# chubbymaggie/syzkaller

Measured on AMD Instinct MI355X. Metric: signal elems triaged/sec (Diff+Merge), higher is better.
Workload: dtype u32

## Files before the change

syzkaller_amd/csrc/agg.hip:

```cpp
#include <algorithm>
#include <utility>
#include <vector>

#include "internal.h"

namespace syz {

constexpr uint32_t kAggThreads = 1024;
constexpr uint32_t kAggSlots = 7424;
constexpr uint32_t kAggBW = 4;
using KBucket = uint4;
constexpr uint32_t kAggBuckets = kAggSlots / kAggBW;
constexpr uint32_t kAggNoSlot = 0xFFFFFFFFu;
static_assert(kAggRegion == kAggSlots, "distinct-list region per partition (internal.h)");
constexpr uint32_t kAggLimit = kAggSlots * 4 / 5;
static_assert(kAggLimit == kAggLimitRecs, "internal.h mirror");
constexpr double kAggTargetLoad = 0.4;
constexpr double kAggTargetLoadEntry = 0.6;
constexpr uint64_t kMinItems = 2048;
constexpr uint32_t kAggEmpty = 0xFFFFFFFFu;
constexpr uint32_t kAggNone = 0xFFFFFFFFu;
constexpr uint32_t kAggOverflow = 0xFFFFFFFFu;
constexpr uint32_t kAggMinBits = 3, kAggMaxBits = 11;
constexpr uint32_t kAggMaxParts = 1u << kAggMaxBits;
constexpr uint32_t kAggTile = 18432;
constexpr uint32_t kAggGroup = 8;
constexpr uint32_t kAggU = 4, kAggD = 2;

struct AggGeom {
	uint32_t pbits;
	uint32_t ibits;
	__host__ __device__ uint32_t rbits() const { return 32 - pbits; }
	__host__ __device__ uint32_t cbits() const { return pbits - 2; }
	__host__ __device__ uint32_t items_per_chunk_log2() const { return cbits() - ibits; }
	__host__ __device__ uint32_t part(uint32_t h) const { return h >> (32 - pbits); }
	__host__ __device__ uint32_t meta(uint32_t level, uint64_t serial) const
	{
		return (level << cbits()) | ((uint32_t)serial & ((1u << cbits()) - 1));
	}
	__host__ __device__ uint32_t rec(uint32_t h, uint32_t meta) const { return (h << pbits) | meta; }
	__host__ __device__ uint32_t resid(uint32_t r) const { return r >> pbits; }
	__host__ __device__ uint32_t level(uint32_t r) const { return (r >> cbits()) & 3; }
	__host__ __device__ uint32_t local(uint32_t r) const { return r & ((1u << cbits()) - 1); }
};

__device__ __forceinline__ uint32_t agg_home_bucket(uint32_t key, const AggGeom& g)
{
	return __umulhi(key << g.pbits, kAggBuckets);
}

__device__ __forceinline__ uint32_t lds_flag(uint32_t* f)
{
	return __hip_atomic_load(f, __ATOMIC_RELAXED, __HIP_MEMORY_SCOPE_WORKGROUP);
}
__device__ __forceinline__ void lds_flag_set(uint32_t* f)
{
	__hip_atomic_store(f, 1u, __ATOMIC_RELAXED, __HIP_MEMORY_SCOPE_WORKGROUP);
}

__device__ __forceinline__ uint32_t bucket_find(uint4 B, uint32_t e)
{
	return B.x == e ? 0 : B.y == e ? 1 : B.z == e ? 2 : B.w == e ? 3 : 4;
}

__device__ __forceinline__ uint32_t bucket_first_empty(uint4 B)
{
	return B.x == kAggEmpty ? 0 : B.y == kAggEmpty ? 1 : B.z == kAggEmpty ? 2 : B.w == kAggEmpty ? 3 : 4;
}

__device__ uint32_t agg_find_insert(KBucket* kb, uint32_t e, uint32_t b, KBucket B, uint32_t* s_ovf, uint32_t& ins)
{
	uint32_t* keys = reinterpret_cast<uint32_t*>(kb);
	for (uint32_t step = 0; step < kAggBuckets;) {
		const uint32_t f = bucket_find(B, e);
		if (f < kAggBW)
			return b * kAggBW + f;
		const uint32_t j = bucket_first_empty(B);
		if (j == kAggBW) {
			b = b + 1 == kAggBuckets ? 0 : b + 1;
			B = kb[b];
			step++;
			continue;
		}
		const uint32_t i = b * kAggBW + j;
		const uint32_t key = atomicCAS(&keys[i], kAggEmpty, e);
		if (key == kAggEmpty) {
			ins++;
			return i;
		}
		if (key == e)
			return i;
		B = kb[b];
	}
	lds_flag_set(s_ovf);
	return kAggNoSlot;
}

struct CellGroup {
	uint64_t ch0;
	uint32_t bnd[kAggGroup + 1];
	__device__ void load(const uint32_t* __restrict__ ot, uint64_t nchunks, uint64_t gi)
	{
		ch0 = gi * kAggGroup;
#pragma unroll
		for (uint32_t i = 0; i <= kAggGroup; i++)
			bnd[i] = ot[min<uint64_t>(ch0 + i, nchunks)];
	}
	__device__ uint32_t serial(uint32_t j, uint32_t r, const AggGeom& g) const
	{
		uint32_t chunk = (uint32_t)ch0;
#pragma unroll
		for (uint32_t i = 1; i < kAggGroup; i++)
			chunk += j >= bnd[i];
		return (chunk << g.cbits()) | g.local(r);
	}
};

template <bool kShard>
__global__ __launch_bounds__(kAggThreads) void k_agg_count(const uint32_t* __restrict__ sigs,
                                                           const uint64_t* __restrict__ call_start,
                                                           const uint32_t* __restrict__ call_len, uint64_t c0,
                                                           uint64_t c1, AggGeom g, AggSrc x, uint32_t* counts)
{
	__shared__ uint32_t h[kAggMaxParts];
	auto add = [&](uint32_t e) {
		if (!kShard || owner_of(e, x.nshards) == x.shard)
			atomicAdd(&h[g.part(fmix32(e))], 1u);
	};
	const uint32_t P = 1u << g.pbits, cb = g.ibits;
	const uint32_t w = threadIdx.x >> 6, nw = blockDim.x >> 6, lane = lane_id();
	const uint64_t ncalls = c1 - c0, nchunks = (ncalls + (1ull << cb) - 1) >> cb;
	for (uint64_t ch = blockIdx.x; ch < nchunks; ch += gridDim.x) {
		for (uint32_t i = threadIdx.x; i < P; i += blockDim.x)
			h[i] = 0;
		__syncthreads();
		const uint64_t ce = min<uint64_t>(ncalls, (ch + 1) << cb);
		for (uint64_t s = (ch << cb) + w; s < ce; s += nw) {
			const uint64_t c = c0 + s, start = call_start[c];
			const uint32_t len = call_len[c];
			uint32_t j = lane;
			for (; j + 192 < len; j += 256) {
				const uint32_t a = sigs[start + j], b = sigs[start + j + 64], d = sigs[start + j + 128],
				               f = sigs[start + j + 192];
				add(a);
				add(b);
				add(d);
				add(f);
			}
			for (; j < len; j += 64)
				add(sigs[start + j]);
		}
		__syncthreads();
		for (uint32_t i = threadIdx.x; i < P; i += blockDim.x)
			counts[ch * P + i] = h[i];
		__syncthreads();
	}
}

__device__ __forceinline__ uint32_t block_excl_scan_1k(uint32_t v, uint32_t* out)
{
	__shared__ uint32_t wsum[16];
	const uint32_t lane = lane_id(), w = threadIdx.x >> 6, nw = blockDim.x >> 6;
	uint32_t x = v;
#pragma unroll
	for (int o = 1; o < 64; o <<= 1) {
		const uint32_t y = __shfl_up(x, o, 64);
		if (lane >= (uint32_t)o)
			x += y;
	}
	if (lane == 63)
		wsum[w] = x;
	__syncthreads();
	uint32_t pre = 0, tot = 0;
	for (uint32_t i = 0; i < nw; i++) {
		pre += i < w ? wsum[i] : 0;
		tot += wsum[i];
	}
	__syncthreads();
	*out = pre + x - v;
	return tot;
}

__global__ __launch_bounds__(1024) void k_agg_scan_chunks(const uint32_t* counts, uint64_t nitems, uint32_t ilog,
                                                          uint32_t P, uint32_t* offs, uint32_t* offsT, uint64_t* totals)
{
	const uint32_t p = blockIdx.x;
	const uint64_t nchunks = (nitems + (1ull << ilog) - 1) >> ilog;
	uint32_t* ot = offsT + (uint64_t)p * (nchunks + 1);
	uint64_t run = 0;
	for (uint64_t b0 = 0; b0 < nitems; b0 += blockDim.x) {
		const uint64_t b = b0 + threadIdx.x;
		const uint32_t v = b < nitems ? counts[b * P + p] : 0;
		uint32_t ex;
		const uint32_t tot = block_excl_scan_1k(v, &ex);
		if (b < nitems) {
			offs[b * P + p] = (uint32_t)(run + ex);
			if ((b & ((1ull << ilog) - 1)) == 0)
				ot[b >> ilog] = (uint32_t)(run + ex);
		}
		run += tot;
	}
	if (threadIdx.x == 0) {
		totals[p] = run;
		ot[nchunks] = (uint32_t)run;
	}
}

__global__ __launch_bounds__(1024) void k_agg_scan_totals(const uint64_t* totals, uint32_t P, uint64_t* rec_base)
{
	__shared__ uint64_t wsum[16];
	const uint32_t lane = lane_id(), w = threadIdx.x >> 6, i0 = threadIdx.x * 2;
	const uint64_t a = i0 < P ? totals[i0] : 0, b = i0 + 1 < P ? totals[i0 + 1] : 0;
	uint64_t x = a + b;
#pragma unroll
	for (int o = 1; o < 64; o <<= 1) {
		const uint64_t y = __shfl_up(x, o, 64);
		if (lane >= (uint32_t)o)
			x += y;
	}
	if (lane == 63)
		wsum[w] = x;
	__syncthreads();
	uint64_t pre = 0, tot = 0;
	for (uint32_t k = 0; k < 16; k++) {
		pre += k < w ? wsum[k] : 0;
		tot += wsum[k];
	}
	const uint64_t ex = pre + x - (a + b);
	if (i0 < P)
		rec_base[i0] = ex;
	if (i0 + 1 < P)
		rec_base[i0 + 1] = ex + a;
	if (threadIdx.x == 0)
		rec_base[P] = tot;
}

constexpr uint32_t kScatChunkMax = 1u << (kAggMaxBits - 2);
constexpr uint32_t kScatWaves = kAggThreads / 64;

constexpr uint32_t kScat3K = 16;
constexpr uint32_t kScat3KEntry = 10;
constexpr uint32_t kScat3Fill = 85;
constexpr uint32_t kScatPer = 12;
constexpr uint32_t kScatPerEntry = 10;
constexpr uint32_t kBlk = 16;
constexpr uint32_t kDummyLines = 2048;
typedef uint32_t scat_v4u __attribute__((ext_vector_type(4)));

struct CapCells {
	const uint64_t* base;
	const uint32_t* cap;
	uint32_t* cnt;
	uint32_t* ovf;
	uint64_t nchunks;
	uint32_t* dummy;
	const uint64_t* sizes = nullptr;
	const uint32_t* tiles = nullptr;
	bool split = false;
	uint32_t tile = 1024;
};

constexpr uint32_t kScat3Tile = kScat3K * 64, kScat3TileEntry = kScat3KEntry * 64;
__host__ __device__ inline uint64_t scat3_tiles(uint32_t len, uint32_t tile)
{
	return (len + tile - 1) / tile;
}
__device__ inline bool scat3_takes(uint64_t recs, uint32_t tiles, uint32_t tile)
{
	return recs * 100 >= (uint64_t)tiles * tile * kScat3Fill;
}

template <bool kOn>
struct PrioLevels {
	uint8_t lvl[kOn ? 256 : 1];
	__device__ __forceinline__ void load(const LevelMap& lm, uint32_t nthreads)
	{
		if (kOn) {
			for (uint32_t i = threadIdx.x; i < 256; i += nthreads)
				lvl[i] = lm.lvl[i];
		}
	}
	__device__ __forceinline__ uint32_t level(uint32_t pv, bool kept, bool& bad) const
	{
		const uint32_t lv = lvl[kOn ? pv : 0];
		bad |= kept && lv == 0xff;
		return lv & 3;
	}
	static __device__ __forceinline__ void report(bool bad, const AggSrc& x)
	{
		if (kOn && x.bad_level && __ballot(bad) && lane_id() == 0)
			atomicOr(x.bad_level, 1u);
	}
};

struct CallTable {
	uint64_t start[kScatChunkMax];
	uint32_t len[kScatChunkMax];
	uint16_t meta[kScatChunkMax];
	template <bool kEntry>
	__device__ __forceinline__ void load(const uint64_t* __restrict__ call_start, const uint32_t* __restrict__ call_len,
	                                     const uint8_t* __restrict__ call_prio, const LevelMap& lm, const AggGeom& g,
	                                     uint64_t c0, uint64_t cbeg, uint32_t nc)
	{
		for (uint32_t i = threadIdx.x; i < nc; i += blockDim.x) {
			const uint64_t c = c0 + cbeg + i;
			start[i] = call_start[c];
			len[i] = call_len[c];
			meta[i] = (uint16_t)g.meta(kEntry ? 0 : lm.lvl[call_prio[c]], cbeg + i);
		}
	}
	__device__ __forceinline__ uint32_t call_of(uint32_t w, uint32_t loc) const { return w + (loc >> 24) * kScatWaves; }
	template <bool kEntry, uint32_t kPer>
	__device__ __forceinline__ uint32_t fetch(uint32_t w, uint32_t lane, uint32_t nc, uint32_t& wc, uint32_t& wo,
	                                          const uint32_t* __restrict__ sigs, const AggSrc& x, uint32_t (&ev)[kPer],
	                                          uint32_t (&loc)[kPer], uint32_t (&pv)[kEntry ? kPer : 1]) const
	{
		constexpr uint32_t kQuota = kPer * 64;
		uint32_t q = 0;
		while (q < kQuota && wc < nc) {
			const uint32_t ln = len[wc], m = min(kQuota - q, ln - wo);
			const uint32_t tag = ((wc - w) / kScatWaves) << 24;
			if (q == 0) {
#pragma unroll
				for (uint32_t u = 0; u < kPer; u++)
					loc[u] = tag | wo;
			}
#pragma unroll
			for (uint32_t u = 0; u < kPer; u++) {
				const uint32_t i = u * 64 + lane;
				loc[u] = i >= q && i < q + m ? tag | (wo + i - q) : loc[u];
			}
			q += m;
			wo += m;
			if (wo == ln) {
				wc += kScatWaves;
				wo = 0;
			}
		}
		if (q) {
#pragma unroll
			for (uint32_t u = 0; u < kPer; u++) {
				const uint64_t a = start[call_of(w, loc[u])] + (loc[u] & 0xFFFFFFu);
				ev[u] = __builtin_nontemporal_load(&sigs[a]);
				if (kEntry)
					pv[kEntry ? u : 0] = (uint8_t)__builtin_nontemporal_load(&x.elem_prio[a]);
			}
		}
		return q;
	}
};

template <bool kEntry>
__global__ __launch_bounds__(kAggThreads) void k_agg_scatter(const uint32_t* __restrict__ sigs,
                                                             const uint64_t* __restrict__ call_start,
                                                             const uint32_t* __restrict__ call_len,
                                                             const uint8_t* __restrict__ call_prio, LevelMap lm,
                                                             uint64_t c0, uint64_t c1, AggGeom g, AggSrc x,
                                                             const uint32_t* __restrict__ offs,
                                                             const uint64_t* __restrict__ rec_base, uint32_t* recs)
{
	constexpr uint32_t kQuota = kAggTile / kScatWaves, kPer = kQuota / 64;
	static_assert(kQuota % 64 == 0, "tile quota per wave");
	__shared__ uint32_t t_rec[kAggTile];
	__shared__ uint16_t t_part[kAggTile];
	__shared__ uint64_t cur[kAggMaxParts];
	__shared__ uint32_t hist[kAggMaxParts], pos[kAggMaxParts];
	__shared__ CallTable calls;
	__shared__ PrioLevels<kEntry> levels;
	const uint32_t P = 1u << g.pbits, cb = g.cbits(), ib = g.ibits;
	levels.load(lm, blockDim.x);
	const uint32_t w = threadIdx.x >> 6, lane = lane_id();
	const uint64_t ncalls = c1 - c0, nitems = (ncalls + (1ull << ib) - 1) >> ib;
	const uint32_t per_t = (P + blockDim.x - 1) / blockDim.x;
	bool badlv = false;
	for (uint64_t ch = blockIdx.x; ch < nitems; ch += gridDim.x) {
		const uint64_t cbeg = ch << ib;
		const uint32_t nc = (uint32_t)min<uint64_t>(ncalls - cbeg, 1ull << ib);
		for (uint32_t i = threadIdx.x; i < P; i += blockDim.x) {
			cur[i] = rec_base[i] + offs[ch * P + i];
			hist[i] = 0;
		}
		calls.load<kEntry>(call_start, call_len, call_prio, lm, g, c0, cbeg, nc);
		__syncthreads();
		uint32_t wc = w, wo = 0;
		uint32_t ev[kPer], loc[kPer], pv[kEntry ? kPer : 1];
		auto fetch = [&]() { return calls.fetch<kEntry>(w, lane, nc, wc, wo, sigs, x, ev, loc, pv); };
		uint32_t n = fetch();
		for (;;) {
#pragma unroll
			for (uint32_t u = 0; u < kPer; u++) {
				const uint32_t i = u * 64 + lane;
				const bool keep = i < n && (!kEntry || x.nshards == 1 || owner_of(ev[u], x.nshards) == x.shard);
				if (keep) {
					const uint32_t h = fmix32(ev[u]), p = g.part(h);
					const uint32_t r = atomicAdd(&hist[p], 1u);
					uint32_t meta = calls.meta[calls.call_of(w, loc[u])];
					if (kEntry)
						meta |= levels.level(pv[kEntry ? u : 0], true, badlv) << cb;
					ev[u] = g.rec(h, meta);
					loc[u] = p | (r << 16);
				} else {
					loc[u] = ~0u;
				}
			}
			__syncthreads();
			uint32_t hsum = 0;
			for (uint32_t q = 0; q < per_t; q++) {
				const uint32_t i = threadIdx.x * per_t + q;
				hsum += i < P ? hist[i] : 0;
			}
			uint32_t ex;
			const uint32_t nt = block_excl_scan_1k(hsum, &ex);
			for (uint32_t q = 0; q < per_t; q++) {
				const uint32_t i = threadIdx.x * per_t + q;
				if (i < P) {
					pos[i] = ex;
					cur[i] -= ex;
					ex += hist[i];
				}
			}
			__syncthreads();
#pragma unroll
			for (uint32_t u = 0; u < kPer; u++) {
				if (loc[u] != ~0u) {
					const uint32_t p = loc[u] & 0xFFFFu, d = pos[p] + (loc[u] >> 16);
					t_rec[d] = ev[u];
					t_part[d] = (uint16_t)p;
				}
			}
			n = fetch();
			__syncthreads();
			for (uint32_t d = threadIdx.x; d < nt; d += blockDim.x)
				recs[cur[t_part[d]] + d] = t_rec[d];
			__syncthreads();
			for (uint32_t i = threadIdx.x; i < P; i += blockDim.x) {
				cur[i] += pos[i] + hist[i];
				hist[i] = 0;
			}
			if (!__syncthreads_or(n != 0))
				break;
		}
	}
	PrioLevels<kEntry>::report(badlv, x);
}

struct ScatLane {
	uint32_t w, lane;
	uint32_t seq = 0;
	bool spilled = false;
};
struct ScatItem {
	uint32_t* recs;
	uint64_t base;
	uint32_t cap;
};
template <uint32_t kB>
struct ScatBlocks {
	static_assert(kB == 16 || kB == 32, "block of 64 or 128 B");
	static constexpr uint32_t kMaxP = kB == 16 ? 2048 : 1024;
	static_assert(kMaxP * kB * 4 == 128 * 1024 && kMaxP <= kAggMaxParts, "128 KB of blocks");
	static constexpr uint32_t kG = 64 / kB;
	static constexpr uint32_t kLB = kB / 4, kGF = 64 / kLB;
	static constexpr uint32_t kShare = (kMaxP + kAggThreads - 1) / kAggThreads;
	alignas(16) uint32_t buf[kMaxP * kB];
	uint32_t fillc[kMaxP + 1];
	uint32_t written[kMaxP + 1];
	uint16_t flist[kShare * kAggThreads];
	uint32_t s_or[2][kScatWaves];

	__device__ __forceinline__ void reset(uint32_t P)
	{
		for (uint32_t i = threadIdx.x; i < P; i += kAggThreads) {
			fillc[i] = 0;
			written[i] = 0;
		}
	}
	__device__ __forceinline__ bool wg_or(ScatLane& t, bool pred)
	{
		uint32_t* r = s_or[t.seq++ & 1];
		const bool any = __ballot(pred) != 0;
		if (t.lane == 0)
			r[t.w] = any;
		__syncthreads();
		return __ballot(r[t.lane & (kScatWaves - 1)] != 0) != 0;
	}
	template <uint32_t M>
	__device__ __forceinline__ uint32_t place(const uint32_t (&rec)[M], const uint32_t (&pt)[M], uint32_t pend)
	{
		uint32_t sl[M];
#pragma unroll
		for (uint32_t u = 0; u < M; u++)
			sl[u] = (pend >> u) & 1 ? atomicAdd(&fillc[pt[u]], 1u) : kB;
#pragma unroll
		for (uint32_t u = 0; u < M; u++) {
			if (sl[u] < kB) {
				buf[pt[u] * kB + sl[u]] = rec[u];
				pend &= ~(1u << u);
			}
		}
		return pend;
	}
	__device__ __forceinline__ void flush(ScatLane& t, uint32_t P, const ScatItem& it, uint32_t* dummy)
	{
		const uint32_t fgrp = t.lane / kLB, fq = t.lane % kLB;
		uint16_t* wl = flist + t.w * kShare * 64;
		uint32_t nw = 0;
#pragma unroll
		for (uint32_t i = 0; i < kShare; i++) {
			const uint32_t p = i * kAggThreads + t.w * 64 + t.lane;
			const bool f = p < P && fillc[p] >= kB;
			const uint64_t m = __ballot(f);
			if (f)
				wl[nw + lane_rank(m)] = (uint16_t)p;
			nw += (uint32_t)__popcll(m);
		}
		for (uint32_t jb = 0; jb < nw; jb += kGF) {
			const bool ok = jb + fgrp < nw;
			const uint32_t pp = wl[min(jb + fgrp, nw - 1)];
			const uint32_t wr = written[pp];
			const scat_v4u v = *reinterpret_cast<const scat_v4u*>(&buf[pp * kB + fq * 4]);
			const bool fits = wr + kB <= it.cap;
			t.spilled |= ok && !fits;
			uint32_t* d = ok && fits ? it.recs + it.base + (uint64_t)pp * it.cap + wr
			                         : dummy + (blockIdx.x % (kDummyLines * kBlk / kB)) * kB;
			*reinterpret_cast<scat_v4u*>(d + fq * 4) = v;
			__builtin_amdgcn_wave_barrier();
			if (fq == 0 && ok) {
				written[pp] = wr + kB;
				fillc[pp] = 0;
			}
		}
	}
	template <uint32_t M>
	__device__ __forceinline__ void scatter_tile(ScatLane& t, uint32_t P, const ScatItem& it, uint32_t* dummy,
	                                             const uint32_t (&rec)[M], const uint32_t (&pt)[M], uint32_t pend)
	{
		for (;;) {
			pend = place(rec, pt, pend);
			const bool more = wg_or(t, pend != 0);
			flush(t, P, it, dummy);
			if (!more)
				break;
			__syncthreads();
		}
	}
	__device__ __forceinline__ void finish(ScatLane& t, uint32_t P, const ScatItem& it, const CapCells& cc, uint64_t ch)
	{
		const uint32_t grp = t.lane / kB, slot = t.lane & (kB - 1);
		for (uint32_t p = t.w * kG + grp; p < P; p += kScatWaves * kG) {
			const uint32_t c = fillc[p], wr = written[p];
			if (wr + c > it.cap)
				t.spilled = true;
			else if (slot < c)
				it.recs[it.base + (uint64_t)p * it.cap + wr + slot] = buf[p * kB + slot];
			if (slot == 0)
				cc.cnt[(uint64_t)p * cc.nchunks + ch] = min(wr + c, it.cap);
		}
		if (t.spilled)
			*cc.ovf = 1u;
		__syncthreads();
	}
};

template <bool kEntry, uint32_t kB>
__global__ __launch_bounds__(kAggThreads, 4) void k_agg_scatter_blk(const uint32_t* __restrict__ sigs,
                                                                    const uint64_t* __restrict__ call_start,
                                                                    const uint32_t* __restrict__ call_len,
                                                                    const uint8_t* __restrict__ call_prio, LevelMap lm,
                                                                    uint64_t c0, uint64_t c1, AggGeom g, AggSrc x,
                                                                    CapCells cc, uint32_t* recs)
{
	constexpr uint32_t kPer = kEntry ? kScatPerEntry : kScatPer;
// ... 63 lines not shown
		return;
	bool badlv = false;
	levels.load(lm, kAggThreads);
	for (uint64_t ch = blockIdx.x; ch < nchunks; ch += gridDim.x) {
		const uint64_t cbeg = ch << g.ibits;
		const uint32_t nc = (uint32_t)min<uint64_t>(ncalls - cbeg, 1ull << g.ibits);
		if (cc.split && !scat3_takes(cc.sizes[ch], cc.tiles[ch], cc.tile))
			continue;
		const ScatItem it{recs, cc.base[ch], cc.cap[ch]};
		blocks.reset(P);
		__syncthreads();
		uint32_t j = w, wo = 0, clen = 0, cmeta = 0;
		uint64_t cstart = 0;
		auto open_call = [&]() {
			while (j < nc) {
				const uint64_t c = c0 + cbeg + j;
				clen = call_len[c];
				if (clen) {
					cstart = call_start[c];
					const uintptr_t pa = (uintptr_t)(call_prio + c);
					const uint32_t word =
					    *(const __attribute__((address_space(4))) uint32_t*)(pa & ~(uintptr_t)3);
					cmeta = g.meta(kEntry ? 0 : levels.lvl[(word >> (8 * (pa & 3))) & 0xFF], cbeg + j);
					return;
				}
				j += kScatWaves;
			}
		};
		open_call();
		auto fetch = [&](uint32_t (&v)[kK], uint32_t (&pv)[kEntry ? kK : 1], uint32_t& n, uint32_t& meta) {
			n = j < nc ? min(kTile, clen - wo) : 0u;
			meta = cmeta;
			const uint32_t* src = sigs + cstart + wo;
			const uint32_t last = n ? n - 1 : 0;
#pragma unroll
			for (uint32_t u = 0; u < kK; u++)
				v[u] = __builtin_nontemporal_load(&src[min(u * 64 + lane, last)]);
			if constexpr (kEntry) {
				const int8_t* psrc = x.elem_prio + cstart + wo;
#pragma unroll
				for (uint32_t u = 0; u < kK; u++)
					pv[u] = (uint8_t)__builtin_nontemporal_load(&psrc[min(u * 64 + lane, last)]);
			}
			if (n) {
				wo += n;
				if (wo == clen) {
					wo = 0;
					j += kScatWaves;
					open_call();
				}
			}
		};
		auto tile = [&](const uint32_t (&v)[kK], const uint32_t (&pv)[kEntry ? kK : 1], uint32_t n, uint32_t meta) {
			uint32_t rec[kK], pt[kK];
#pragma unroll
			for (uint32_t u = 0; u < kK; u++) {
				const uint32_t h = fmix32(v[u]);
				pt[u] = g.part(h);
				uint32_t m = meta;
				if constexpr (kEntry)
					m |= levels.level(pv[kEntry ? u : 0], u * 64 + lane < n, badlv) << g.cbits();
				rec[u] = g.rec(h, m);
			}
			const uint32_t nu = n > lane ? (n - lane + 63) >> 6 : 0u;
			blocks.scatter_tile(t, P, it, cc.dummy, rec, pt, (1u << nu) - 1);
		};
		uint32_t va[kK], vb[kK], pa[kEntry ? kK : 1], pb[kEntry ? kK : 1], na, nb, ma, mb;
		fetch(va, pa, na, ma);
		for (;;) {
			fetch(vb, pb, nb, mb);
			tile(va, pa, na, ma);
			if (!blocks.wg_or(t, nb != 0))
				break;
			fetch(va, pa, na, ma);
			tile(vb, pb, nb, mb);
			if (!blocks.wg_or(t, na != 0))
				break;
		}
		blocks.finish(t, P, it, cc, ch);
	}
	PrioLevels<kEntry>::report(badlv, x);
}

static uint64_t nchunks_of(uint64_t ncalls, uint32_t ibits)
{
	return (ncalls + (1ull << ibits) - 1) >> ibits;
}

static void launch_capped_scatter(hipStream_t s, const syzsig_batch* b, uint64_t c0, uint64_t c1, const LevelMap& lm,
                                  const AggGeom& g, CapCells cc, uint32_t* recs, const AggSrc* xp)
{
	const uint32_t grid = (uint32_t)std::min<uint64_t>(cc.nchunks, 2048);
	const bool wide = g.pbits < kAggMaxBits;
	const AggSrc x = xp ? *xp : AggSrc{nullptr, 1, 0, 0};
	auto launch = [&](auto kernel, auto... tail) {
		kernel<<<grid, kAggThreads, 0, s>>>(b->sigs, b->call_start, b->call_len, b->call_prio, lm, c0, c1, g, tail...);
	};
	if (!xp || xp->nshards == 1) {
		cc.split = xp || (cc.sizes && cc.tiles);
		if (!xp)
			launch(k_scat3<kScat3K, false, 16>, cc, recs, x);
		else if (wide)
			launch(k_scat3<kScat3KEntry, true, 32>, cc, recs, x);
		else
			launch(k_scat3<kScat3KEntry, true, 16>, cc, recs, x);
		if (!cc.split)
			return;
	}
	if (xp)
		launch(wide ? k_agg_scatter_blk<true, 32> : k_agg_scatter_blk<true, 16>, x, cc, recs);
	else
		launch(wide ? k_agg_scatter_blk<false, 32> : k_agg_scatter_blk<false, 16>, x, cc, recs);
}

__global__ __launch_bounds__(256) void k_chunk_sizes(const uint32_t* __restrict__ call_len, uint64_t c0, uint64_t c1,
                                                     uint32_t cbits, uint64_t* sizes, uint32_t* tiles, uint32_t tile)
{
	const uint64_t ch = blockIdx.x, cbeg = c0 + (ch << cbits), cend = min<uint64_t>(c1, cbeg + (1ull << cbits));
	uint64_t s = 0, t = 0;
	for (uint64_t c = cbeg + threadIdx.x; c < cend; c += blockDim.x) {
		s += call_len[c];
		t += scat3_tiles(call_len[c], tile);
	}
	s = wave_sum_u64(s);
	t = wave_sum_u64(t);
	__shared__ uint64_t ws[4][2];
	if (lane_id() == 0) {
		ws[threadIdx.x >> 6][0] = s;
		ws[threadIdx.x >> 6][1] = t;
	}
	__syncthreads();
	if (threadIdx.x == 0) {
		sizes[ch] = ws[0][0] + ws[1][0] + ws[2][0] + ws[3][0];
		if (tiles)
			tiles[ch] = (uint32_t)min<uint64_t>(ws[0][1] + ws[1][1] + ws[2][1] + ws[3][1], 0xFFFFFFFFu);
	}
}

__device__ __forceinline__ void cell_plan(const uint64_t* __restrict__ sizes, uint64_t nchunks, uint32_t P, float sd,
                                          uint64_t* base, uint32_t* cap)
{
	__shared__ uint64_t wsum[16];
	uint64_t run = 0;
	for (uint64_t b0 = 0; b0 < nchunks; b0 += blockDim.x) {
		const uint64_t c = b0 + threadIdx.x;
		uint64_t v = 0;
		if (c < nchunks) {
			const float m = (float)sizes[c] / (float)P;
			const uint32_t k = sd < 0 ? 64u : ((uint32_t)(m + sd * sqrtf(m)) + 64 + 63) & ~63u;
			cap[c] = k;
			v = (uint64_t)k * P;
		}
		uint64_t xs = v;
		const uint32_t lane = lane_id(), w = threadIdx.x >> 6;
#pragma unroll
		for (int o = 1; o < 64; o <<= 1) {
			const uint64_t y = __shfl_up(xs, o, 64);
			if (lane >= (uint32_t)o)
				xs += y;
		}
		if (lane == 63)
			wsum[w] = xs;
		__syncthreads();
		uint64_t pre = 0, tot = 0;
		for (uint32_t i = 0; i < 16; i++) {
			pre += i < w ? wsum[i] : 0;
			tot += wsum[i];
		}
		if (c < nchunks)
			base[c] = run + pre + xs - v;
		run += tot;
		__syncthreads();
	}
}

__global__ __launch_bounds__(1024) void k_cell_plan(const uint64_t* __restrict__ sizes, uint64_t nchunks, uint32_t P,
                                                    float sd, uint64_t* base, uint32_t* cap)
{
	cell_plan(sizes, nchunks, P, sd, base, cap);
}

__global__ __launch_bounds__(256) void k_fast_prep(const uint64_t* __restrict__ call_start,
                                                   const uint32_t* __restrict__ call_len,
                                                   const uint8_t* __restrict__ call_prio, uint64_t c0, uint64_t c1,
                                                   uint32_t ibits, uint64_t nrec_space, uint64_t* sizes,
                                                   uint64_t* part, uint8_t* call_new, LevelMap lm, uint32_t* tiles)
{
	const uint64_t ch = blockIdx.x, cbeg = c0 + (ch << ibits), cend = min<uint64_t>(c1, cbeg + (1ull << ibits));
	uint64_t tot = 0, bad = 0, other = 0, nt = 0;
	for (uint64_t c = cbeg + threadIdx.x; c < cend; c += blockDim.x) {
		const uint64_t st = call_start[c];
		const uint32_t ln = call_len[c];
		tot += ln;
		nt += scat3_tiles(ln, kScat3Tile);
		bad += st > nrec_space || ln > nrec_space - st || ln > kSerialMask;
		other |= lm.lvl[call_prio[c]] == 0xff;
		call_new[c] = 0;
	}
	tot = wave_sum_u64(tot);
	bad = wave_sum_u64(bad);
	other = wave_sum_u64(other);
	nt = wave_sum_u64(nt);
	__shared__ uint64_t ws[4][4];
	if (lane_id() == 0) {
		ws[threadIdx.x >> 6][0] = tot;
		ws[threadIdx.x >> 6][1] = bad;
		ws[threadIdx.x >> 6][2] = other;
		ws[threadIdx.x >> 6][3] = nt;
	}
	__syncthreads();
	if (threadIdx.x == 0) {
		uint64_t t = 0, b = 0, o = 0, tl = 0;
		for (int w = 0; w < 4; w++) {
			t += ws[w][0];
			b += ws[w][1];
			o += ws[w][2];
			tl += ws[w][3];
		}
		sizes[ch] = t;
		if (tiles)
			tiles[ch] = (uint32_t)min<uint64_t>(tl, 0xFFFFFFFFu);
		part[2 * ch] = t;
		part[2 * ch + 1] = b | (o ? 1ull << 63 : 0);
	}
}

__global__ __launch_bounds__(1024) void k_cell_plan_fast(const uint64_t* __restrict__ sizes, uint64_t nchunks,
                                                         uint32_t P, float sd, uint64_t* base, uint32_t* cap,
                                                         const uint64_t* __restrict__ part, uint64_t guess,
                                                         uint64_t npairs0, unsigned long long* ctr)
{
	__shared__ unsigned long long s_tot, s_flag;
	if (threadIdx.x == 0) {
		s_tot = 0;
		s_flag = 0;
	}
	if (threadIdx.x < kNumCounters)
		ctr[threadIdx.x] = threadIdx.x == kCntAux2 ? npairs0 : 0;
	__syncthreads();
	uint64_t t = 0, f = 0;
	for (uint64_t c = threadIdx.x; c < nchunks; c += blockDim.x) {
		t += part[2 * c];
		f |= part[2 * c + 1];
	}
	t = wave_sum_u64(t);
	for (int o = 32; o > 0; o >>= 1)
		f |= __shfl_xor(f, o, 64);
	if (lane_id() == 0) {
		atomicAdd(&s_tot, (unsigned long long)t);
		atomicOr(&s_flag, (unsigned long long)f);
	}
	__syncthreads();
	if (threadIdx.x == 0) {
		ctr[kCntRecords] = s_tot;
		ctr[kCntSpill] = (s_flag >> 63 ? 2u : 0u) | ((s_flag & ~(1ull << 63)) || s_tot > guess ? 4u : 0u);
	}
	cell_plan(sizes, nchunks, P, sd, base, cap);
}

struct AggLds {
	KBucket kb[kAggBuckets];
	uint32_t fl[4][kAggSlots];
	uint2 q[kAggThreads / 64][64];
	uint32_t s_n, s_ovf, s_out, s_next;
};

struct AggCells {
	const uint32_t* recs;
	const uint64_t* rec_base;
	const uint32_t* offsT;
	const uint64_t* cap_base;
	const uint32_t* cap_len;
	const uint32_t* cap_cnt;
	uint64_t nchunks;
	uint32_t ilog, gsz;
	const uint32_t* spill;
	unsigned long long* ctr;
};

template <uint32_t U, uint32_t D, bool kCap, bool kIdx32>
__device__ __forceinline__ bool agg_partition(AggLds& L, uint32_t p, const AggCells& x, const AggGeom& g)
{
	KBucket* kb = L.kb;
	auto& fl = L.fl;
	const uint32_t* __restrict__ recs = x.recs;
	const uint64_t* __restrict__ rec_base = x.rec_base;
	const uint32_t* __restrict__ offsT = x.offsT;
	const uint64_t* __restrict__ cap_base = x.cap_base;
	const uint32_t* __restrict__ cap_len = x.cap_len;
	const uint32_t* __restrict__ cap_cnt = x.cap_cnt;
	const uint64_t nchunks = x.nchunks;
	const uint32_t ilog = x.ilog, gsz = x.gsz;
	const uint32_t lane = lane_id();
	uint2* wq = L.q[threadIdx.x >> 6];
	uint32_t qn = 0;
	auto flush_queue = [&]() {
		uint32_t ins = 0;
		if (lds_flag(&L.s_ovf)) {
			qn = 0;
			return;
		}
		if (lane < qn) {
			const uint2 e = wq[lane];
			const uint32_t hb = __umulhi(e.x << g.pbits, kAggBuckets);
			const uint32_t slot = agg_find_insert(kb, e.x, hb, kb[hb], &L.s_ovf, ins);
			if (slot != kAggNoSlot)
				atomicMin(&fl[e.y >> 24][slot], e.y & 0xFFFFFFu);
		}
		const uint32_t n_ins = (uint32_t)wave_sum_u64(ins);
		if (n_ins && lane == 0 && atomicAdd(&L.s_n, n_ins) + n_ins > kAggLimit)
			lds_flag_set(&L.s_ovf);
		qn = 0;
		__builtin_amdgcn_wave_barrier();
	};
	const uint64_t ngroups = (nchunks + gsz - 1) / gsz;
	for (uint32_t i = threadIdx.x; i < kAggSlots; i += blockDim.x) {
		if (i < kAggSlots)
			reinterpret_cast<uint32_t*>(kb)[i] = kAggEmpty;
		fl[0][i] = fl[1][i] = fl[2][i] = fl[3][i] = kAggNone;
	}
	if (threadIdx.x == 0) {
		L.s_n = 0;
		L.s_ovf = 0;
		L.s_out = 0;
		L.s_next = 0;
	}
	__syncthreads();
	const uint32_t* ot = offsT + (uint64_t)p * (nchunks + 1);
	for (;;) {
		uint32_t gi = 0;
		if (lane == 0)
			gi = atomicAdd(&L.s_next, 1u);
		gi = __builtin_amdgcn_readfirstlane(__shfl(gi, 0, 64));
		if (gi >= ngroups || lds_flag(&L.s_ovf))
			break;
		const uint64_t ch0 = (uint64_t)gi * gsz;
		uint64_t lbase = 0;
		uint32_t llen = 0;
		{
			const uint64_t c = ch0 + lane;
			if (lane < gsz && c < nchunks) {
				if (kCap) {
					lbase = cap_base[c] + (uint64_t)p * cap_len[c];
					llen = cap_cnt[(uint64_t)p * nchunks + c];
				} else {
					lbase = rec_base[p] + ot[c];
					llen = ot[c + 1] - ot[c];
				}
			}
		}
		uint32_t lvs = llen;
#pragma unroll
		for (uint32_t o = 1; o < 64; o <<= 1) {
			if (o < gsz) {
				const uint32_t y = __shfl_up(lvs, o, 64);
				if (lane >= o)
					lvs += y;
			}
		}
		const uint32_t n = __builtin_amdgcn_readlane(lvs, gsz - 1);
		if (n == 0)
			continue;
		lvs -= llen;
		const uint64_t ldelta = lbase - lvs;
		const uint32_t nl = n - 1;
		auto cells = [&](uint32_t o0, uint32_t& c0, uint64_t& inside) {
			c0 = (uint32_t)__popcll(__ballot(lane < gsz && lvs <= o0)) - 1;
			inside = __ballot(lane < gsz && lvs > o0 && lvs < o0 + U * 64);
		};
		auto delta_of = [&](uint32_t i) -> uint64_t {
			const uint32_t lo = __builtin_amdgcn_readlane((uint32_t)ldelta, i);
			const uint32_t hi = __builtin_amdgcn_readlane((uint32_t)(ldelta >> 32), i);
			return (uint64_t)hi << 32 | lo;
		};
		auto fetch = [&](uint32_t (&buf)[U], uint32_t o0) {
			uint32_t c0;
			uint64_t inside;
			cells(min(o0, nl), c0, inside);
			if constexpr (kIdx32) {
				const uint32_t d0 = __builtin_amdgcn_readlane((uint32_t)ldelta, c0);
				uint32_t v[U], d[U];
#pragma unroll
				for (uint32_t u = 0; u < U; u++) {
					v[u] = min(o0 + u * 64 + lane, nl);
					d[u] = d0;
				}
				for (uint64_t m = inside; m; m &= m - 1) {
					const uint32_t j = __builtin_ctzll(m), vs = __builtin_amdgcn_readlane(lvs, j);
					const uint32_t dj = __builtin_amdgcn_readlane((uint32_t)ldelta, j);
#pragma unroll
					for (uint32_t u = 0; u < U; u++)
						d[u] = v[u] >= vs ? dj : d[u];
				}
#pragma unroll
				for (uint32_t u = 0; u < U; u++)
					buf[u] = __builtin_nontemporal_load(&recs[v[u] + d[u]]);
				return;
			}
			const uint64_t d0 = delta_of(c0);
			uint32_t v[U];
			uint64_t d[U];
#pragma unroll
			for (uint32_t u = 0; u < U; u++) {
				v[u] = min(o0 + u * 64 + lane, nl);
				d[u] = d0;
			}
			for (uint64_t m = inside; m; m &= m - 1) {
				const uint32_t j = __builtin_ctzll(m), vs = __builtin_amdgcn_readlane(lvs, j);
				const uint64_t dj = delta_of(j);
#pragma unroll
				for (uint32_t u = 0; u < U; u++)
					d[u] = v[u] >= vs ? dj : d[u];
			}
#pragma unroll
			for (uint32_t u = 0; u < U; u++)
				buf[u] = __builtin_nontemporal_load(&recs[v[u] + d[u]]);
		};
		auto absorb = [&](const uint32_t (&buf)[U], uint32_t o0) {
			uint32_t c0;
			uint64_t inside;
			cells(o0, c0, inside);
			uint32_t key[U], lv[U], k[U], hb[U], slot[U], c[U];
#pragma unroll
			for (uint32_t u = 0; u < U; u++)
				c[u] = (uint32_t)ch0 + c0;
			for (uint64_t m = inside; m; m &= m - 1) {
				const uint32_t vs = __builtin_amdgcn_readlane(lvs, __builtin_ctzll(m));
#pragma unroll
				for (uint32_t u = 0; u < U; u++)
					c[u] += min(o0 + u * 64 + lane, nl) >= vs;
			}
#pragma unroll
			for (uint32_t u = 0; u < U; u++) {
				const uint32_t r = buf[u];
				k[u] = ((c[u] >> ilog) << g.cbits()) | g.local(r);
				key[u] = g.resid(r);
				lv[u] = g.level(r);
				hb[u] = __umulhi(r & ~((1u << g.pbits) - 1), kAggBuckets);
			}
			KBucket B[U];
#pragma unroll
			for (uint32_t u = 0; u < U; u++)
				B[u] = kb[hb[u]];
			bool any_need = false;
#pragma unroll
			for (uint32_t u = 0; u < U; u++) {
				const uint32_t f = bucket_find(B[u], key[u]);
				slot[u] = f < kAggBW ? hb[u] * kAggBW + f : kAggNoSlot;
				any_need |= f >= kAggBW;
			}
			if (__builtin_amdgcn_readfirstlane((uint32_t)(__ballot(any_need) != 0))) {
#pragma unroll
				for (uint32_t u = 0; u < U; u++) {
					const bool nd = slot[u] == kAggNoSlot;
					const uint64_t m = __ballot(nd);
					if (!m)
						continue;
					const uint32_t c = (uint32_t)__popcll(m);
					if (qn + c > 64)
						flush_queue();
					if (nd)
						wq[qn + lane_rank(m)] = make_uint2(key[u], (lv[u] << 24) | k[u]);
					qn += c;
				}
				__builtin_amdgcn_wave_barrier();
			}
#pragma unroll
			for (uint32_t u = 0; u < U; u++)
				if (slot[u] != kAggNoSlot)
					atomicMin(&fl[lv[u]][slot[u]], k[u]);
		};
		uint32_t buf[D + 1][U];
#pragma unroll
		for (uint32_t d = 0; d < D; d++)
			fetch(buf[d], d * U * 64);
		bool more = true;
		for (uint32_t o0 = 0; more;) {
#pragma unroll
			for (uint32_t t = 0; t <= D; t++) {
				if (more) {
					fetch(buf[(t + D) % (D + 1)], o0 + D * U * 64);
					absorb(buf[t], o0);
					o0 += U * 64;
					more = o0 < n;
				}
			}
		}
	}
	flush_queue();
	__syncthreads();
	return !L.s_ovf;
}

template <uint32_t U, uint32_t D, bool kCap, bool kIdx32 = false>
__global__ __launch_bounds__(kAggThreads) void k_agg(AggCells x, AggGeom g, uint32_t* dist_e, uint4* dist_f,
                                                     uint32_t* cnt)
{
	__shared__ AggLds L;
	const uint32_t* keys = reinterpret_cast<const uint32_t*>(L.kb);
	const uint32_t P = 1u << g.pbits, lane = lane_id();
	if (x.spill && *x.spill)
		return;
	for (uint32_t p = blockIdx.x; p < P; p += gridDim.x) {
		if (!agg_partition<U, D, kCap, kIdx32>(L, p, x, g)) {
			if (threadIdx.x == 0) {
				cnt[p] = kAggOverflow;
				if (x.ctr)
					atomicAdd(&x.ctr[kCntAggOvf], 1ull);
			}
			__syncthreads();
			continue;
		}
		const uint32_t hp = p << g.rbits();
		for (uint32_t i0 = 0; i0 < kAggSlots; i0 += kAggThreads) {
			const uint32_t i = i0 + threadIdx.x;
			const uint32_t key = i < kAggSlots ? keys[i] : kAggEmpty;
			const bool occ = key != kAggEmpty;
			const uint64_t m = __ballot(occ);
			uint32_t wb = 0;
			if (lane == 0 && m)
				wb = atomicAdd(&L.s_out, (uint32_t)__popcll(m));
			wb = __shfl(wb, 0, 64);
			if (occ) {
				const uint64_t o = (uint64_t)p * kAggRegion + wb + lane_rank(m);
				dist_e[o] = fmix32_inv(hp | key);
				dist_f[o] = make_uint4(L.fl[0][i], L.fl[1][i], L.fl[2][i], L.fl[3][i]);
			}
		}
		__syncthreads();
		if (threadIdx.x == 0) {
			cnt[p] = L.s_out;
			if (x.ctr && L.s_out)
				atomicAdd(&x.ctr[kCntDistinct], (unsigned long long)L.s_out);
		}
		__syncthreads();
	}
}

template <bool kCap>
static void launch_agg(const syzsig_ctx* ctx, uint64_t extent, uint32_t P, hipStream_t s, const AggCells& xc,
                       const AggGeom& g, void* de, void* df, void* dc)
{
	if (extent <= (1ull << 32) && !(ctx->agg_dbg & SYZSIG_DEBUG_AGG_IDX64))
		k_agg<kAggU, kAggD, kCap, true><<<P, kAggThreads, 0, s>>>(xc, g, (uint32_t*)de, (uint4*)df, (uint32_t*)dc);
	else
		k_agg<kAggU, kAggD, kCap, false><<<P, kAggThreads, 0, s>>>(xc, g, (uint32_t*)de, (uint4*)df, (uint32_t*)dc);
}

__global__ __launch_bounds__(256) void k_agg_global(const uint32_t* __restrict__ recs,
                                                    const uint64_t* __restrict__ rec_base,
                                                    const uint32_t* __restrict__ offsT, uint64_t nchunks, AggGeom g,
                                                    const uint32_t* __restrict__ ovl, uint32_t novl, uint32_t* gkeys,
                                                    uint32_t* gfl, uint64_t C, unsigned long long* err)
{
	const uint32_t lane = lane_id();
	const uint64_t ngroups = (nchunks + kAggGroup - 1) / kAggGroup, items = (uint64_t)novl * ngroups;
	const uint64_t nwaves = (uint64_t)gridDim.x * (blockDim.x >> 6);
	uint64_t bad = 0;
	for (uint64_t it = blockIdx.x * (uint64_t)(blockDim.x >> 6) + (threadIdx.x >> 6); it < items; it += nwaves) {
		const uint32_t p = ovl[it / ngroups];
		const uint32_t* ot = offsT + (uint64_t)p * (nchunks + 1);
		const uint32_t* pr = recs + rec_base[p];
		CellGroup cg;
		cg.load(ot, nchunks, it % ngroups);
		for (uint32_t j = cg.bnd[0] + lane; j < cg.bnd[kAggGroup]; j += 64) {
			const uint32_t r = pr[j];
			const uint32_t k = cg.serial(j, r, g), l = g.level(r);
			const uint32_t h = (p << g.rbits()) | g.resid(r);
			uint64_t i = C;
			if (h != kAggEmpty) {
				i = fmix32(h ^ 0x632BE5ABu) & (C - 1);
				for (uint64_t step = 0;; step++) {
					uint32_t key = gkeys[i];
					if (key == kAggEmpty) {
						key = atomicCAS(&gkeys[i], kAggEmpty, h);
						if (key == kAggEmpty)
							break;
					}
					if (key == h)
						break;
					i = (i + 1) & (C - 1);
					if (step >= C) {
						bad++;
						i = ~0ull;
						break;
					}
				}
			}
			if (i != ~0ull)
				atomicMin(&gfl[(uint64_t)l * (C + 1) + i], k);
		}
	}
	block_count(err, bad);
}

__global__ __launch_bounds__(256) void k_agg_global_compact(const uint32_t* __restrict__ gkeys,
                                                            const uint32_t* __restrict__ gfl, uint64_t C,
                                                            uint32_t* dist_e, uint4* dist_f,
                                                            unsigned long long* out_cnt)
{
	const uint32_t lane = lane_id();
	for (uint64_t i0 = blockIdx.x * (uint64_t)blockDim.x; i0 <= C; i0 += (uint64_t)gridDim.x * blockDim.x) {
		const uint64_t i = i0 + threadIdx.x;
		bool occ = false;
		uint32_t h = kAggEmpty;
		uint4 f = make_uint4(kAggNone, kAggNone, kAggNone, kAggNone);
		if (i <= C) {
			f = make_uint4(gfl[i], gfl[(C + 1) + i], gfl[2 * (C + 1) + i], gfl[3 * (C + 1) + i]);
			if (i < C) {
				h = gkeys[i];
				occ = h != kAggEmpty;
			} else {
				occ = (f.x & f.y & f.z & f.w) != kAggNone;
			}
		}
		const uint64_t m = __ballot(occ);
		unsigned long long wb = 0;
		if (lane == 0 && m)
			wb = atomicAdd(out_cnt, (unsigned long long)__popcll(m));
		wb = __shfl(wb, 0, 64);
		if (occ) {
			dist_e[wb + lane_rank(m)] = fmix32_inv(h);
			dist_f[wb + lane_rank(m)] = f;
		}
	}
}

constexpr uint32_t kFinThreads = 256, kFinBuf = 4 * kFinThreads * 2, kFinIlp = 2;

__global__ __launch_bounds__(kFinThreads) void k_agg_finalize(const uint32_t* __restrict__ dist_e,
                                                              const uint4* __restrict__ dist_f,
                                                              const uint32_t* __restrict__ cnt, uint32_t nregions,
                                                              LevelMap lm, uint64_t c0, uint64_t* slots,
                                                              uint64_t bmask, uint64_t* ns_slots, uint64_t ns_bmask,
                                                              uint8_t* call_new, uint64_t* pairs,
                                                              unsigned long long* npairs, unsigned long long* ctr)
{
	__shared__ uint64_t buf[kFinBuf];
	__shared__ uint32_t s_n;
	__shared__ unsigned long long s_base;
	const uint64_t max_probe = max_probe_for(bmask);
	uint64_t inserted = 0, changed = 0, ns_ins = 0, ovf = 0;
	if (threadIdx.x == 0)
		s_n = 0;
	__syncthreads();
	auto flush = [&](uint32_t nb) {
		nb = min(nb, kFinBuf);
		if (threadIdx.x == 0)
			s_base = atomicAdd(npairs, (unsigned long long)nb);
		__syncthreads();
		for (uint32_t t = threadIdx.x; t < nb; t += blockDim.x)
			pairs[s_base + t] = buf[t];
		__syncthreads();
		if (threadIdx.x == 0)
			s_n = 0;
		__syncthreads();
	};
	auto emit = [&](uint64_t v) {
		const uint32_t k = atomicAdd(&s_n, 1u);
		if (k < kFinBuf)
			buf[k] = v;
		else
			pairs[atomicAdd(npairs, 1ull)] = v;
	};
	for (uint32_t r = blockIdx.x; r < nregions; r += gridDim.x) {
		const uint32_t n = cnt[r] == kAggOverflow ? 0 : cnt[r];
		for (uint32_t i0 = 0; i0 < n; i0 += kFinIlp * kFinThreads) {
			uint32_t e[kFinIlp];
			uint4 f4[kFinIlp];
			int top[kFinIlp];
#pragma unroll
			for (uint32_t k = 0; k < kFinIlp; k++) {
				const uint32_t i = i0 + k * kFinThreads + threadIdx.x;
				const uint64_t o = (uint64_t)r * kAggRegion + min(i, n - 1);
				e[k] = dist_e[o];
				f4[k] = dist_f[o];
				top[k] = -1;
				const uint32_t f[4] = {f4[k].x, f4[k].y, f4[k].z, f4[k].w};
#pragma unroll
				for (int l = 0; l < 4; l++)
					if (i < n && l < (int)lm.n && f[l] != kAggNone)
						top[k] = l;
			}
			Bucket bm[kFinIlp], bn[kFinIlp];
#pragma unroll
			for (uint32_t k = 0; k < kFinIlp; k++) {
				if (top[k] >= 0) {
					bm[k] = load_bucket(slots + (home_bucket(e[k], bmask) << kBucketShift));
					if (ns_slots)
						bn[k] = load_bucket(ns_slots + (home_bucket(e[k], ns_bmask) << kBucketShift));
				}
			}
#pragma unroll
			for (uint32_t k = 0; k < kFinIlp; k++) {
				if (top[k] < 0)
					continue;
				const uint32_t f[4] = {f4[k].x, f4[k].y, f4[k].z, f4[k].w};
				const int8_t P = lm.val[top[k]];
				const uint64_t word = make_slot(e[k], P);
				uint64_t old = 0;
				const int64_t idx = tbl_find_or_insert_from(slots, bmask, e[k], word, old, max_probe, bm[k]);
				if (idx < 0) {
					ovf++;
					continue;
				}
				const bool present = slot_live(old);
				const int p0 = present ? (int)slot_prio(old) : -1000;
				if ((int)P <= p0)
					continue;
				if (old != 0)
					slots[idx] = word;
				inserted += !present;
				changed++;
				const int rr = tbl_merge_from(ns_slots, ns_bmask, e[k], P, bn[k]);
				ns_ins += rr == 1;
				ovf += rr < 0;
				uint32_t mk = kAggNone;
#pragma unroll
				for (int l = 3; l >= 0; l--) {
					if (l > top[k] || f[l] == kAggNone)
						continue;
					if ((int)lm.val[l] <= p0)
						break;
					if (f[l] < mk) {
						mk = f[l];
						const uint64_t c = c0 + f[l];
						call_new[c] = 1;
						emit((c << 32) | e[k]);
					}
				}
			}
			__syncthreads();
			const uint32_t nb = s_n;
			if (nb > kFinBuf / 2)
				flush(nb);
		}
	}
	__syncthreads();
	const uint32_t nb = s_n;
	if (nb)
		flush(nb);
	block_count(&ctr[kCntInserted], inserted);
	block_count(&ctr[kCntChanged], changed);
	block_count(&ctr[kCntAux], ns_ins);
	block_count(&ctr[kCntOverflow], ovf);
}

constexpr uint32_t kFxThreads = 512, kFxSet = 8192, kFxBuf = 2048, kFxProbe = 64;
enum : int { kFxTaken = 0, kFxClaimed = 1, kFxFull = 2 };

__device__ __forceinline__ int fx_claim(uint32_t* set, uint32_t tag, uint64_t rel)
{
	const uint32_t key = (tag << 31) | (uint32_t)(rel + 1);
	uint32_t h = fmix32(key) & (kFxSet - 1);
	for (uint32_t step = 0; step < kFxProbe; step++) {
		uint32_t v = set[h];
		if (v == 0) {
			v = atomicCAS(&set[h], 0u, key);
			if (v == 0)
				return kFxClaimed;
		}
		if (v == key)
			return kFxTaken;
		h = (h + 1) & (kFxSet - 1);
	}
	return kFxFull;
}

__device__ __forceinline__ int64_t fx_walk(const uint64_t* tab, uint64_t b, uint64_t bend, uint64_t slice0,
                                           uint32_t e, Bucket B, uint32_t* set, uint32_t tag, uint64_t& old)
{
	for (uint64_t b0 = b; b < bend; b++) {
		if (b != b0)
			B = load_bucket(tab + (b << kBucketShift));
#pragma unroll
		for (uint32_t i = 0; i < kBucketSlots; i++) {
			const uint64_t sw = B.s[i], idx = (b << kBucketShift) + i;
			if (sw != kSlotEmpty) {
				if (slot_key(sw) == e) {
					old = sw;
					return (int64_t)idx;
				}
				continue;
			}
			const int c = fx_claim(set, tag, idx - slice0);
// ... 1407 lines not shown
```

Measured before the change: 277.3 billion.

## Add single-chunk fast path to aggregation fetch/absorb and simplify slot addressing

In the 32-bit-index path, the fetch step now caches the current chunk boundary and delta. When a whole U*64 window falls inside one chunk, it uses a contiguous base pointer and passes a precomputed chunk key to absorb. Absorb then skips the per-window ballot/readlane cell search. Bucket hashing now uses a fixed-shift multiply, and the flag atomicMin address is computed as a precomputed byte offset. The extra state adds register pressure, and a guard is added so scat3_takes handles zero tiles.

After: 289.1 billion, median of 6. 4.3% higher.

```diff
diff --git a/syzkaller_amd/csrc/agg.hip b/syzkaller_amd/csrc/agg.hip
--- a/syzkaller_amd/csrc/agg.hip
+++ b/syzkaller_amd/csrc/agg.hip
@@ -1,4 +1,5 @@
 #include <algorithm>
+#include <type_traits>
 #include <utility>
 #include <vector>
 
@@ -12,6 +13,7 @@
 using KBucket = uint4;
 constexpr uint32_t kAggBuckets = kAggSlots / kAggBW;
 constexpr uint32_t kAggNoSlot = 0xFFFFFFFFu;
+constexpr uint32_t kAggNoChunk = 0xFFFFFFFFu;
 static_assert(kAggRegion == kAggSlots, "distinct-list region per partition (internal.h)");
 constexpr uint32_t kAggLimit = kAggSlots * 4 / 5;
 static_assert(kAggLimit == kAggLimitRecs, "internal.h mirror");
@@ -44,9 +46,15 @@
 	__host__ __device__ uint32_t local(uint32_t r) const { return r & ((1u << cbits()) - 1); }
 };
 
-__device__ __forceinline__ uint32_t agg_home_bucket(uint32_t key, const AggGeom& g)
-{
-	return __umulhi(key << g.pbits, kAggBuckets);
+static_assert(((uint64_t)kAggBuckets << kAggMaxBits) < (1u << 24), "24-bit multiply");
+__device__ __forceinline__ uint32_t agg_home_bucket(uint32_t r)
+{
+	return __umulhi(r >> kAggMaxBits, kAggBuckets << kAggMaxBits);
+}
+
+__device__ __forceinline__ uint64_t ballot64(bool b)
+{
+	return __builtin_amdgcn_ballot_w64(b);
 }
 
 __device__ __forceinline__ uint32_t lds_flag(uint32_t* f)
@@ -267,7 +275,7 @@
 }
 __device__ inline bool scat3_takes(uint64_t recs, uint32_t tiles, uint32_t tile)
 {
-	return recs * 100 >= (uint64_t)tiles * tile * kScat3Fill;
+	return tiles && recs * 100 >= (uint64_t)tiles * tile * kScat3Fill;
 }
 
 template <bool kOn>
@@ -937,7 +945,7 @@
 		}
 		if (lane < qn) {
 			const uint2 e = wq[lane];
-			const uint32_t hb = __umulhi(e.x << g.pbits, kAggBuckets);
+			const uint32_t hb = agg_home_bucket(e.x << g.pbits);
 			const uint32_t slot = agg_find_insert(kb, e.x, hb, kb[hb], &L.s_ovf, ins);
 			if (slot != kAggNoSlot)
 				atomicMin(&fl[e.y >> 24][slot], e.y & 0xFFFFFFu);
@@ -999,22 +1007,46 @@
 		lvs -= llen;
 		const uint64_t ldelta = lbase - lvs;
 		const uint32_t nl = n - 1;
+		uint32_t f_next = 0, f_kc = 0;
+		uint64_t f_delta = 0;
 		auto cells = [&](uint32_t o0, uint32_t& c0, uint64_t& inside) {
-			c0 = (uint32_t)__popcll(__ballot(lane < gsz && lvs <= o0)) - 1;
-			inside = __ballot(lane < gsz && lvs > o0 && lvs < o0 + U * 64);
+			c0 = (uint32_t)__popcll(ballot64(lane < gsz && lvs <= o0)) - 1;
+			inside = ballot64(lane < gsz && lvs > o0 && lvs < o0 + U * 64);
 		};
 		auto delta_of = [&](uint32_t i) -> uint64_t {
 			const uint32_t lo = __builtin_amdgcn_readlane((uint32_t)ldelta, i);
 			const uint32_t hi = __builtin_amdgcn_readlane((uint32_t)(ldelta >> 32), i);
 			return (uint64_t)hi << 32 | lo;
 		};
-		auto fetch = [&](uint32_t (&buf)[U], uint32_t o0) {
-			uint32_t c0;
-			uint64_t inside;
-			cells(min(o0, nl), c0, inside);
+		auto fetch = [&](uint32_t (&buf)[U], uint32_t& kc, uint32_t o0) {
+			const uint32_t* a[U];
+			kc = kAggNoChunk;
+			bool one_cell = false;
 			if constexpr (kIdx32) {
-				const uint32_t d0 = __builtin_amdgcn_readlane((uint32_t)ldelta, c0);
-				uint32_t v[U], d[U];
+				if (o0 >= f_next) {
+					const uint32_t oc = min(o0, nl);
+					const uint32_t c = (uint32_t)__popcll(ballot64(lane < gsz && lvs <= oc)) - 1;
+					const uint64_t later = ballot64(lane < gsz && lvs > oc);
+					f_next = later ? __builtin_amdgcn_readlane(lvs, __builtin_ctzll(later)) : n;
+					f_delta = delta_of(c);
+					f_kc = ((((uint32_t)ch0 + c) >> ilog) << g.cbits());
+				}
+				one_cell = o0 + U * 64 <= f_next;
+			}
+			if (one_cell) {
+				const uint32_t* sb = recs + (f_delta + o0);
+#pragma unroll
+				for (uint32_t u = 0; u < U; u++)
+					a[u] = sb + (lane + u * 64);
+				kc = f_kc;
+			} else {
+				uint32_t c0;
+				uint64_t inside;
+				cells(min(o0, nl), c0, inside);
+				using Delta = std::conditional_t<kIdx32, uint32_t, uint64_t>;
+				const Delta d0 = (Delta)delta_of(c0);
+				uint32_t v[U];
+				Delta d[U];
 #pragma unroll
 				for (uint32_t u = 0; u < U; u++) {
 					v[u] = min(o0 + u * 64 + lane, nl);
@@ -1022,73 +1054,67 @@
 				}
 				for (uint64_t m = inside; m; m &= m - 1) {
 					const uint32_t j = __builtin_ctzll(m), vs = __builtin_amdgcn_readlane(lvs, j);
-					const uint32_t dj = __builtin_amdgcn_readlane((uint32_t)ldelta, j);
+					const Delta dj = (Delta)delta_of(j);
 #pragma unroll
 					for (uint32_t u = 0; u < U; u++)
 						d[u] = v[u] >= vs ? dj : d[u];
 				}
 #pragma unroll
 				for (uint32_t u = 0; u < U; u++)
-					buf[u] = __builtin_nontemporal_load(&recs[v[u] + d[u]]);
-				return;
-			}
-			const uint64_t d0 = delta_of(c0);
-			uint32_t v[U];
-			uint64_t d[U];
-#pragma unroll
-			for (uint32_t u = 0; u < U; u++) {
-				v[u] = min(o0 + u * 64 + lane, nl);
-				d[u] = d0;
-			}
-			for (uint64_t m = inside; m; m &= m - 1) {
-				const uint32_t j = __builtin_ctzll(m), vs = __builtin_amdgcn_readlane(lvs, j);
-				const uint64_t dj = delta_of(j);
+					a[u] = &recs[(Delta)(v[u] + d[u])];
+			}
+#pragma unroll
+			for (uint32_t u = 0; u < U; u++)
+				buf[u] = __builtin_nontemporal_load(a[u]);
+		};
+		auto absorb = [&](const uint32_t (&buf)[U], uint32_t kc, uint32_t o0) {
+			uint32_t key[U], lv[U], k[U], hb[U], at[U];
+			bool found[U];
+			if (kIdx32 && kc != kAggNoChunk) {
 #pragma unroll
 				for (uint32_t u = 0; u < U; u++)
-					d[u] = v[u] >= vs ? dj : d[u];
-			}
-#pragma unroll
-			for (uint32_t u = 0; u < U; u++)
-				buf[u] = __builtin_nontemporal_load(&recs[v[u] + d[u]]);
-		};
-		auto absorb = [&](const uint32_t (&buf)[U], uint32_t o0) {
-			uint32_t c0;
-			uint64_t inside;
-			cells(o0, c0, inside);
-			uint32_t key[U], lv[U], k[U], hb[U], slot[U], c[U];
-#pragma unroll
-			for (uint32_t u = 0; u < U; u++)
-				c[u] = (uint32_t)ch0 + c0;
-			for (uint64_t m = inside; m; m &= m - 1) {
-				const uint32_t vs = __builtin_amdgcn_readlane(lvs, __builtin_ctzll(m));
+					k[u] = kc | g.local(buf[u]);
+			} else {
+				uint32_t c0, c[U];
+				uint64_t inside;
+				cells(o0, c0, inside);
 #pragma unroll
 				for (uint32_t u = 0; u < U; u++)
-					c[u] += min(o0 + u * 64 + lane, nl) >= vs;
+					c[u] = (uint32_t)ch0 + c0;
+				for (uint64_t m = inside; m; m &= m - 1) {
+					const uint32_t vs = __builtin_amdgcn_readlane(lvs, __builtin_ctzll(m));
+#pragma unroll
+					for (uint32_t u = 0; u < U; u++)
+						c[u] += min(o0 + u * 64 + lane, nl) >= vs;
+				}
+#pragma unroll
+				for (uint32_t u = 0; u < U; u++)
+					k[u] = ((c[u] >> ilog) << g.cbits()) | g.local(buf[u]);
 			}
 #pragma unroll
 			for (uint32_t u = 0; u < U; u++) {
 				const uint32_t r = buf[u];
-				k[u] = ((c[u] >> ilog) << g.cbits()) | g.local(r);
 				key[u] = g.resid(r);
 				lv[u] = g.level(r);
-				hb[u] = __umulhi(r & ~((1u << g.pbits) - 1), kAggBuckets);
+				hb[u] = agg_home_bucket(r);
 			}
 			KBucket B[U];
 #pragma unroll
 			for (uint32_t u = 0; u < U; u++)
 				B[u] = kb[hb[u]];
-			bool any_need = false;
+			uint64_t need = 0;
 #pragma unroll
 			for (uint32_t u = 0; u < U; u++) {
-				const uint32_t f = bucket_find(B[u], key[u]);
-				slot[u] = f < kAggBW ? hb[u] * kAggBW + f : kAggNoSlot;
-				any_need |= f >= kAggBW;
-			}
-			if (__builtin_amdgcn_readfirstlane((uint32_t)(__ballot(any_need) != 0))) {
+				const bool m0 = B[u].x == key[u], m1 = B[u].y == key[u], m2 = B[u].z == key[u], m3 = B[u].w == key[u];
+				found[u] = m0 | m1 | m2 | m3;
+				at[u] = lv[u] * (kAggSlots * 4) + hb[u] * (kAggBW * 4) + (m3 ? 12u : m2 ? 8u : m1 ? 4u : 0u);
+				need |= ballot64(!found[u]);
+			}
+			if (need) {
 #pragma unroll
 				for (uint32_t u = 0; u < U; u++) {
-					const bool nd = slot[u] == kAggNoSlot;
-					const uint64_t m = __ballot(nd);
+					const bool nd = !found[u];
+					const uint64_t m = ballot64(nd);
 					if (!m)
 						continue;
 					const uint32_t c = (uint32_t)__popcll(m);
@@ -1102,20 +1128,20 @@
 			}
 #pragma unroll
 			for (uint32_t u = 0; u < U; u++)
-				if (slot[u] != kAggNoSlot)
-					atomicMin(&fl[lv[u]][slot[u]], k[u]);
+				if (found[u])
+					atomicMin(reinterpret_cast<uint32_t*>(reinterpret_cast<char*>(&fl[0][0]) + at[u]), k[u]);
 		};
-		uint32_t buf[D + 1][U];
+		uint32_t buf[D + 1][U], kcr[D + 1];
 #pragma unroll
 		for (uint32_t d = 0; d < D; d++)
-			fetch(buf[d], d * U * 64);
+			fetch(buf[d], kcr[d], d * U * 64);
 		bool more = true;
 		for (uint32_t o0 = 0; more;) {
 #pragma unroll
 			for (uint32_t t = 0; t <= D; t++) {
 				if (more) {
-					fetch(buf[(t + D) % (D + 1)], o0 + D * U * 64);
-					absorb(buf[t], o0);
+					fetch(buf[(t + D) % (D + 1)], kcr[(t + D) % (D + 1)], o0 + D * U * 64);
+					absorb(buf[t], kcr[t], o0);
 					o0 += U * 64;
 					more = o0 < n;
 				}
```
